# tarepan/VectorQuantizedCPC

Measured on AMD Instinct MI355X. Metric: audio samples/sec (WaveRNN-style decode, convert.py path: encode + generate), higher is better.
Workload: dtype f32

## Files before the change

vectorquantizedcpc_amd/csrc/ar_chain.h:

```cpp
#pragma once
#include "ar_xcd.h"
#include "ar_shared.h"

namespace {

constexpr int HR = 896, HF = 256, NC = 256;
constexpr int NW = 32;
constexpr int UPB = 28;
constexpr int ROWS = 3 * UPB;
constexpr int FPB = 8;
constexpr int THREADS = 768;
constexpr int NT_H = HR / 8;
constexpr int NT_A = HF / 8;

__host__ __device__ constexpr int xg_h(int bxt) { return NW * bxt * 32; }
__host__ __device__ constexpr int xg_a(int bxt) { return NW * bxt * FPB; }
__host__ __device__ constexpr int xg_c() { return NW * 16; }
__host__ __device__ constexpr int xg_region(int bxt) { return xg_h(bxt) + xg_a(bxt) + xg_c(); }
constexpr int CTL_WORDS = 64;



template <int STEP>
__device__ __forceinline__ void gran_load1(u64 (&v)[1], const u64 *base, unsigned off) {
    asm volatile("s_nop 4\n\tglobal_load_dwordx2 %0, %1, %2 sc1\n\ts_waitcnt vmcnt(0)" : "=&v"(v[0]) : "v"(off), "s"(base) : "memory");
}
template <int STEP>
__device__ __forceinline__ void gran_load2(u64 (&v)[2], const u64 *base, unsigned off) {
    asm volatile("s_nop 4\n\tglobal_load_dwordx2 %0, %2, %3 sc1\n\tglobal_load_dwordx2 %1, %2, %3 offset:%4 sc1\n\ts_waitcnt vmcnt(0)"
                 : "=&v"(v[0]), "=&v"(v[1]) : "v"(off), "s"(base), "i"(STEP) : "memory");
}
template <int STEP>
__device__ __forceinline__ void gran_load4(u64 (&v)[4], const u64 *base, unsigned off) {
    asm volatile("s_nop 4\n\tglobal_load_dwordx2 %0, %4, %5 sc1\n\tglobal_load_dwordx2 %1, %4, %5 offset:%6 sc1\n\t"
                 "global_load_dwordx2 %2, %4, %5 offset:%7 sc1\n\tglobal_load_dwordx2 %3, %4, %5 offset:%8 sc1\n\ts_waitcnt vmcnt(0)"
                 : "=&v"(v[0]), "=&v"(v[1]), "=&v"(v[2]), "=&v"(v[3]) : "v"(off), "s"(base), "i"(STEP), "i"(2 * STEP), "i"(3 * STEP) : "memory");
}
template <int STEP>
__device__ __forceinline__ void gran_load4b(u64 (&v)[4], const u64 *base, const u64 *base2, unsigned off) {
    asm volatile("s_nop 4\n\tglobal_load_dwordx2 %0, %4, %5 sc1\n\tglobal_load_dwordx2 %1, %4, %5 offset:%7 sc1\n\t"
                 "global_load_dwordx2 %2, %4, %6 sc1\n\tglobal_load_dwordx2 %3, %4, %6 offset:%7 sc1\n\ts_waitcnt vmcnt(0)"
                 : "=&v"(v[0]), "=&v"(v[1]), "=&v"(v[2]), "=&v"(v[3]) : "v"(off), "s"(base), "s"(base2), "i"(STEP) : "memory");
}
template <int STEP>
__device__ __forceinline__ void gran_load8b(u64 (&v)[2][4], const u64 *base, const u64 *base2, unsigned off) {
    asm volatile("s_nop 4\n\tglobal_load_dwordx2 %0, %8, %9 sc1\n\tglobal_load_dwordx2 %1, %8, %9 offset:%11 sc1\n\t"
                 "global_load_dwordx2 %2, %8, %10 sc1\n\tglobal_load_dwordx2 %3, %8, %10 offset:%11 sc1\n\t"
                 "global_load_dwordx2 %4, %8, %9 offset:128 sc1\n\tglobal_load_dwordx2 %5, %8, %9 offset:%12 sc1\n\t"
                 "global_load_dwordx2 %6, %8, %10 offset:128 sc1\n\tglobal_load_dwordx2 %7, %8, %10 offset:%12 sc1\n\ts_waitcnt vmcnt(0)"
                 : "=&v"(v[0][0]), "=&v"(v[0][1]), "=&v"(v[0][2]), "=&v"(v[0][3]), "=&v"(v[1][0]), "=&v"(v[1][1]), "=&v"(v[1][2]), "=&v"(v[1][3])
                 : "v"(off), "s"(base), "s"(base2), "i"(STEP), "i"(STEP + 128) : "memory");
}
template <int N, int STEP>
__device__ __forceinline__ void gran_load_pair(u64 (&a)[N], u64 (&b)[N], const u64 *base, unsigned off, unsigned off2) {
    if constexpr (N == 1)
        asm volatile("s_nop 4\n\tglobal_load_dwordx2 %0, %2, %4 sc1\n\tglobal_load_dwordx2 %1, %3, %4 sc1\n\ts_waitcnt vmcnt(0)"
                     : "=&v"(a[0]), "=&v"(b[0]) : "v"(off), "v"(off2), "s"(base) : "memory");
    if constexpr (N == 2)
        asm volatile("s_nop 4\n\tglobal_load_dwordx2 %0, %4, %6 sc1\n\tglobal_load_dwordx2 %1, %4, %6 offset:%7 sc1\n\t"
                     "global_load_dwordx2 %2, %5, %6 sc1\n\tglobal_load_dwordx2 %3, %5, %6 offset:%7 sc1\n\ts_waitcnt vmcnt(0)"
                     : "=&v"(a[0]), "=&v"(a[1]), "=&v"(b[0]), "=&v"(b[1]) : "v"(off), "v"(off2), "s"(base), "i"(STEP) : "memory");
    if constexpr (N == 4)
        asm volatile("s_nop 4\n\tglobal_load_dwordx2 %0, %8, %10 sc1\n\tglobal_load_dwordx2 %1, %8, %10 offset:%11 sc1\n\t"
                     "global_load_dwordx2 %2, %8, %10 offset:%12 sc1\n\tglobal_load_dwordx2 %3, %8, %10 offset:%13 sc1\n\t"
                     "global_load_dwordx2 %4, %9, %10 sc1\n\tglobal_load_dwordx2 %5, %9, %10 offset:%11 sc1\n\t"
                     "global_load_dwordx2 %6, %9, %10 offset:%12 sc1\n\tglobal_load_dwordx2 %7, %9, %10 offset:%13 sc1\n\ts_waitcnt vmcnt(0)"
                     : "=&v"(a[0]), "=&v"(a[1]), "=&v"(a[2]), "=&v"(a[3]), "=&v"(b[0]), "=&v"(b[1]), "=&v"(b[2]), "=&v"(b[3])
                     : "v"(off), "v"(off2), "s"(base), "i"(STEP), "i"(2 * STEP), "i"(3 * STEP) : "memory");
}
template <int N, int STEP>
__device__ __forceinline__ void gran_load(u64 (&v)[N], const u64 *base, unsigned off) {
    if constexpr (N == 1) gran_load1<STEP>(v, base, off);
    if constexpr (N == 2) gran_load2<STEP>(v, base, off);
    if constexpr (N == 4) gran_load4<STEP>(v, base, off);
}

#define XD_QP(J) "quad_perm:[" #J "," #J "," #J "," #J "] row_mask:0xf bank_mask:0xf"
#define XD_FMAC8(J)                                                                                                      \
    asm("v_fmac_f32_dpp %0, %1, %9 " XD_QP(J) "\n\tv_fmac_f32_dpp %0, %2, %10 " XD_QP(J) "\n\t"                        \
        "v_fmac_f32_dpp %0, %3, %11 " XD_QP(J) "\n\tv_fmac_f32_dpp %0, %4, %12 " XD_QP(J) "\n\t"                       \
        "v_fmac_f32_dpp %0, %5, %13 " XD_QP(J) "\n\tv_fmac_f32_dpp %0, %6, %14 " XD_QP(J) "\n\t"                       \
        "v_fmac_f32_dpp %0, %7, %15 " XD_QP(J) "\n\tv_fmac_f32_dpp %0, %8, %16 " XD_QP(J)                              \
        : "+v"(acc)                                                                                                      \
        : "v"(h[0]), "v"(h[1]), "v"(h[2]), "v"(h[3]), "v"(h[4]), "v"(h[5]), "v"(h[6]), "v"(h[7]),                       \
          "v"(w[0]), "v"(w[1]), "v"(w[2]), "v"(w[3]), "v"(w[4]), "v"(w[5]), "v"(w[6]), "v"(w[7]))
#define XD_FMAC4(J)                                                                                                      \
    asm("v_fmac_f32_dpp %0, %1, %5 " XD_QP(J) "\n\tv_fmac_f32_dpp %0, %2, %6 " XD_QP(J) "\n\t"                         \
        "v_fmac_f32_dpp %0, %3, %7 " XD_QP(J) "\n\tv_fmac_f32_dpp %0, %4, %8 " XD_QP(J)                                \
        : "+v"(acc)                                                                                                      \
        : "v"(h[0]), "v"(h[1]), "v"(h[2]), "v"(h[3]), "v"(w[0]), "v"(w[1]), "v"(w[2]), "v"(w[3]))
template <int J>
__device__ __forceinline__ void fmac8(float &acc, const float *h, const float *w) {
    if constexpr (J == 0) XD_FMAC8(0);
    if constexpr (J == 1) XD_FMAC8(1);
    if constexpr (J == 2) XD_FMAC8(2);
    if constexpr (J == 3) XD_FMAC8(3);
}
template <int J>
__device__ __forceinline__ void fmac4(float &acc, const float *h, const float *w) {
    if constexpr (J == 0) XD_FMAC4(0);
    if constexpr (J == 1) XD_FMAC4(1);
    if constexpr (J == 2) XD_FMAC4(2);
    if constexpr (J == 3) XD_FMAC4(3);
}
template <int LEN>
__device__ __forceinline__ void chain_phase(float &acc, const float (&hv)[8], const float *w) {
    if constexpr (LEN == 32) { fmac8<0>(acc, hv, w); fmac8<1>(acc, hv, w + 8); fmac8<2>(acc, hv, w + 16); fmac8<3>(acc, hv, w + 24); }
    else { fmac4<0>(acc, hv, w); fmac4<1>(acc, hv, w + 4); fmac4<2>(acc, hv, w + 8); fmac4<3>(acc, hv, w + 12); }
}

template <int NT>
__device__ __forceinline__ int phase_pos_t(int n) { return (NT % 32 != 0 && n >= NT - NT % 32) ? n : ((n & ~31) + ((n >> 2) & 1) * 16 + ((n >> 3) & 3) * 4 + (n & 3)); }
template <int NT>
__device__ __forceinline__ float chain_regs(const float *w, const float *opnd) {
    float acc = 0.f;
    constexpr int NPH = (NT + 31) / 32;
    float4 cur[2], nxt[2];
    cur[0] = *(const float4 *)opnd; cur[1] = *(const float4 *)(opnd + 16);
#pragma unroll
    for (int ph = 0; ph < NPH; ++ph) {
        const int len = NT - 32 * ph < 32 ? NT - 32 * ph : 32;
        if (ph + 1 < NPH) {
            const int nlen = NT - 32 * (ph + 1) < 32 ? NT - 32 * (ph + 1) : 32;
            nxt[0] = *(const float4 *)(opnd + 32 * (ph + 1));
            nxt[1] = nlen == 32 ? *(const float4 *)(opnd + 32 * (ph + 1) + 16) : nxt[0];
        }
        const float hv[8] = {cur[0].x, cur[0].y, cur[0].z, cur[0].w, cur[1].x, cur[1].y, cur[1].z, cur[1].w};
        if (len == 32) chain_phase<32>(acc, hv, w + 32 * ph);
        else chain_phase<16>(acc, hv, w + 32 * ph);
        cur[0] = nxt[0]; cur[1] = nxt[1];
    }
    return acc;
}
__device__ __forceinline__ void load_phase(const float *opnd, int ph, int nlen, float4 (&d)[2]) {
    d[0] = *(const float4 *)(opnd + 32 * ph);
    d[1] = nlen == 32 ? *(const float4 *)(opnd + 32 * ph + 16) : d[0];
}
template <int NT, int WS>
__device__ __forceinline__ void chain_lds2(const float4 *wp, const float4 (&w0)[8], const float *opA, const float *opB, bool two,
                                           float &accA, float &accB) {
    constexpr int NPH = (NT + 31) / 32;
    float4 curA[2], nxtA[2], curB[2], nxtB[2], wc[8], wn[8];
    load_phase(opA, 0, NT < 32 ? NT : 32, curA);
    if (two) load_phase(opB, 0, NT < 32 ? NT : 32, curB);
    else { curB[0] = curA[0]; curB[1] = curA[1]; }
#pragma unroll
    for (int i = 0; i < 8; ++i) wc[i] = w0[i];
    accA = 0.f; accB = 0.f;
#pragma unroll
    for (int ph = 0; ph < NPH; ++ph) {
        const int len = NT - 32 * ph < 32 ? NT - 32 * ph : 32;
        if (ph + 1 < NPH) {
            const int nlen = NT - 32 * (ph + 1) < 32 ? NT - 32 * (ph + 1) : 32;
            load_phase(opA, ph + 1, nlen, nxtA);
            if (two) load_phase(opB, ph + 1, nlen, nxtB);
#pragma unroll
            for (int i = 0; i < nlen / 4; ++i) wn[i] = wp[(8 * (ph + 1) + i) * WS];
        }
        __builtin_amdgcn_sched_barrier(0);
        float wv[32];
#pragma unroll
        for (int i = 0; i < 8; ++i) { wv[4 * i] = wc[i].x; wv[4 * i + 1] = wc[i].y; wv[4 * i + 2] = wc[i].z; wv[4 * i + 3] = wc[i].w; }
        {
            const float hv[8] = {curA[0].x, curA[0].y, curA[0].z, curA[0].w, curA[1].x, curA[1].y, curA[1].z, curA[1].w};
            if (len == 32) chain_phase<32>(accA, hv, wv);
            else chain_phase<16>(accA, hv, wv);
        }
        if (two) {
            const float hv[8] = {curB[0].x, curB[0].y, curB[0].z, curB[0].w, curB[1].x, curB[1].y, curB[1].z, curB[1].w};
            if (len == 32) chain_phase<32>(accB, hv, wv);
            else chain_phase<16>(accB, hv, wv);
        }
        __builtin_amdgcn_sched_barrier(0);
        curA[0] = nxtA[0]; curA[1] = nxtA[1]; curB[0] = nxtB[0]; curB[1] = nxtB[1];
#pragma unroll
        for (int i = 0; i < 8; ++i) wc[i] = wn[i];
    }
}

__device__ __forceinline__ unsigned xd_lane_of(unsigned rr, unsigned cc) { return 16u * (2u * (rr >> 2) + (cc & 1u)) + 4u * (cc >> 1) + (rr & 3u); }

__device__ __forceinline__ float chain_combine(float acc) {
    const auto sw = __builtin_amdgcn_permlane16_swap(__float_as_uint(acc), __float_as_uint(acc), false, false);
    const float o = __uint_as_float(sw[1]);
    const float q = acc + o;
    float s;
    asm("s_nop 1\n\tv_add_f32_dpp %0, %1, %1 row_shl:4 row_mask:0xf bank_mask:0xf\n\t"
        "v_add_f32_dpp %0, %1, %0 row_shl:8 row_mask:0xf bank_mask:0xf\n\t"
        "v_add_f32_dpp %0, %1, %0 row_shl:12 row_mask:0xf bank_mask:0xf" : "=&v"(s) : "v"(q));
    return s;
}

template <int NS>
__device__ __forceinline__ int chain_pos(int k, int stride) {
    const int S = k >> 4, kw = S / NS, s = S - kw * NS;
    const int q = (k >> 2) & 3, c0 = k & 1, ci = (k >> 1) & 1;
    return (2 * kw + c0) * stride + phase_pos_t<8 * NS>(8 * s + 4 * ci + q);
}

typedef float v4f __attribute__((ext_vector_type(4)));
constexpr int HS4 = HR + 4;
constexpr int NG_H = NT_H / 8;
template <int NS>
__device__ __forceinline__ int chain_pos_plain(int k, int stride) {
    const int S = k >> 4, kw = S / NS, s = S - kw * NS;
    const int q = (k >> 2) & 3, c0 = k & 1, ci = (k >> 1) & 1;
    return (2 * kw + c0) * stride + 8 * s + 4 * ci + q;
}
template <int G0, int G1>
__device__ __forceinline__ void chain_mfma_regs(v4f &acc, const float *w, const float *op, float4 (&cur)[2]) {
    float4 nxt[2];
#pragma unroll
    for (int g = G0; g < G1; ++g) {
        nxt[0] = cur[0]; nxt[1] = cur[1];
        const float hv[8] = {cur[0].x, cur[0].y, cur[0].z, cur[0].w, cur[1].x, cur[1].y, cur[1].z, cur[1].w};
        __builtin_amdgcn_sched_barrier(0);
#pragma unroll
        for (int i = 0; i < 8; ++i) acc = __builtin_amdgcn_mfma_f32_4x4x1f32(w[8 * g + i], hv[i], acc, 0, 0, 0);
        if (g + 1 < NG_H) { nxt[0] = *(const float4 *)(op + 8 * (g + 1)); nxt[1] = *(const float4 *)(op + 8 * (g + 1) + 4); }
        __builtin_amdgcn_sched_barrier(0);
        cur[0] = nxt[0]; cur[1] = nxt[1];
    }
}
template <int WS, int D>
__device__ __forceinline__ v4f chain_mfma_lds(const float4 *wp, const float4 *wpre, const float *op) {
    v4f acc = {0.f, 0.f, 0.f, 0.f};
    float4 hb[D][2], wb[D][2];
#pragma unroll
    for (int d = 0; d < D; ++d) {
        hb[d][0] = *(const float4 *)(op + 8 * d); hb[d][1] = *(const float4 *)(op + 8 * d + 4);
        wb[d][0] = wpre[2 * d]; wb[d][1] = wpre[2 * d + 1];
    }
#pragma unroll
    for (int g = 0; g < NG_H; ++g) {
        const int s = g % D;
        __builtin_amdgcn_sched_barrier(0);
        const float hv[8] = {hb[s][0].x, hb[s][0].y, hb[s][0].z, hb[s][0].w, hb[s][1].x, hb[s][1].y, hb[s][1].z, hb[s][1].w};
        const float wv[8] = {wb[s][0].x, wb[s][0].y, wb[s][0].z, wb[s][0].w, wb[s][1].x, wb[s][1].y, wb[s][1].z, wb[s][1].w};
#pragma unroll
        for (int i = 0; i < 8; ++i) acc = __builtin_amdgcn_mfma_f32_4x4x1f32(wv[i], hv[i], acc, 0, 0, 0);
        __builtin_amdgcn_sched_barrier(0);
        if (g + D < NG_H) {
            hb[s][0] = *(const float4 *)(op + 8 * (g + D)); hb[s][1] = *(const float4 *)(op + 8 * (g + D) + 4);
            wb[s][0] = wp[(2 * (g + D)) * WS]; wb[s][1] = wp[(2 * (g + D) + 1) * WS];
        }
    }
    return acc;
}

}
```

vectorquantizedcpc_amd/csrc/ar_xcd.hip:

```cpp
#include "ar_xcd.h"
#include "ar_shared.h"

#ifdef VQCPC_XD_STAMPS
__device__ unsigned long long g_xd_stamps[128 * 16];
#define XD_STAMP(wv, i) do { if (rank == 5 && xcc == 0 && wave == (wv) && lane == 0 && t >= 256 && t < 384) \
        g_xd_stamps[(t - 256) * 16 + (i)] = __builtin_amdgcn_s_memrealtime(); } while (0)
extern "C" int vqcpc_debug_xd_stamps(unsigned long long *out) {
    return hipMemcpyFromSymbol(out, HIP_SYMBOL(g_xd_stamps), sizeof(g_xd_stamps)) == hipSuccess ? 0 : -1;
}
__device__ unsigned long long g_xd_workers[6 * 32 * 128];
#define XD_WSTAMP(ev) do { if (xcc == 0 && lane == 0 && t >= 256 && t < 384) \
        g_xd_workers[((ev) * 32 + rank) * 128 + (t - 256)] = __builtin_amdgcn_s_memrealtime(); } while (0)
extern "C" int vqcpc_debug_xd_workers(unsigned long long *out) {
    return hipMemcpyFromSymbol(out, HIP_SYMBOL(g_xd_workers), sizeof(g_xd_workers)) == hipSuccess ? 0 : -1;
}
#else
#define XD_STAMP(wv, i) do { } while (0)
#define XD_WSTAMP(ev) do { } while (0)
#endif
#ifdef VQCPC_XD_BARS
__device__ unsigned long long g_xd_bars[128 * 12 * 4];
#define XD_BARRIVE() do { xd_arrived = __builtin_amdgcn_s_memrealtime(); } while (0)
#define XD_BLEAVE(i) do { if (rank == 5 && xcc == 0 && lane == 0 && t >= 256 && t < 384) { \
        g_xd_bars[((t - 256) * 12 + wave) * 4 + (i)] = xd_arrived; \
        g_xd_bars[((t - 256) * 12 + wave) * 4 + (i) + 1] = __builtin_amdgcn_s_memrealtime(); } } while (0)
extern "C" int vqcpc_debug_xd_bars(unsigned long long *out) {
    return hipMemcpyFromSymbol(out, HIP_SYMBOL(g_xd_bars), sizeof(g_xd_bars)) == hipSuccess ? 0 : -1;
}
#else
#define XD_BARRIVE() do { } while (0)
#define XD_BLEAVE(i) do { } while (0)
#endif

#include "ar_chain.h"

#ifndef XD_ABLATE
#define XD_ABLATE 0
#endif
#ifndef XD_GSPLIT
#define XD_GSPLIT 10
#endif
#ifndef XD_DEPTH
#define XD_DEPTH 3
#endif
#ifndef XD_HOLD
#define XD_HOLD 1
#endif

namespace {

template <int BXT> struct Lds {
    static constexpr int gemb = 0;
    static constexpr int fc1w = gemb + NC * ROWS;
    static constexpr int fc2w = fc1w + FPB * HR;
    static constexpr int whx = fc2w + FPB * HF;
    static constexpr int HS = BXT == 4 ? HS4 : HR;
    static constexpr int hc = whx + 4 * HR;
    static constexpr int ac = hc + BXT * HS;
    static constexpr int gsum = ac + BXT * 8 * 48;
    static constexpr int noise = gsum + BXT * 96;
    static constexpr int mtab = noise + 2 * BXT * 8;
    static constexpr int bq = mtab + NC;
    static constexpr int seg = bq + 96;
    static constexpr int sinfo = seg + BXT * 8;
    static constexpr int ctl = sinfo + BXT * 2;
    static constexpr int total = ctl + 8;
};

template <int BXT, bool RESUME>
__device__ __forceinline__ void xcd_decoder(const XdParams &p, const XdResume &rp) {
    extern __shared__ __attribute__((aligned(16))) float smem[];
    using L = Lds<BXT>;
    float *gemb = smem + L::gemb, *fc1w = smem + L::fc1w, *fc2w = smem + L::fc2w, *whx = smem + L::whx, *hc = smem + L::hc,
          *ac = smem + L::ac, *gsum = smem + L::gsum;
    float *noise = smem + L::noise, *mtab = smem + L::mtab, *c_bq = smem + L::bq;
    int *seg_st = (int *)(smem + L::seg), *sinfo = (int *)(smem + L::sinfo), *s_ctl = (int *)(smem + L::ctl);

    const unsigned tid = threadIdx.x, lane = tid & 63u;
    const int wave = __builtin_amdgcn_readfirstlane((int)(tid >> 6));

    if (tid == 0) {
        unsigned xid;
        asm volatile("s_getreg_b32 %0, hwreg(HW_REG_XCC_ID)" : "=s"(xid));
        xid &= 7u;
        if (p.dbg_misplace && blockIdx.x == 0) xid = (xid + 1u) & 7u;
        unsigned *ctl = (unsigned *)p.xg;
        const unsigned r = __hip_atomic_fetch_add(ctl + xid, 1u, __ATOMIC_RELAXED, __HIP_MEMORY_SCOPE_AGENT);
        __hip_atomic_fetch_add(ctl + 8, 1u, __ATOMIC_RELAXED, __HIP_MEMORY_SCOPE_AGENT);
        int ok = 1;
        const u64 t0 = __builtin_amdgcn_s_memrealtime();
        for (unsigned spins = 0; __hip_atomic_load(ctl + 8, __ATOMIC_RELAXED, __HIP_MEMORY_SCOPE_AGENT) < gridDim.x; ++spins) {
            if ((spins & 63) == 63 && (__builtin_amdgcn_s_memrealtime() - t0 > (u64)p.timeout_ticks ||
                                       __hip_atomic_load(p.status, __ATOMIC_RELAXED, __HIP_MEMORY_SCOPE_SYSTEM) != 0u)) { ok = 0; break; }
            __builtin_amdgcn_s_sleep(2);
        }
        if (ok)
            for (int x = 0; x < 8; ++x)
                if (__hip_atomic_load(ctl + x, __ATOMIC_RELAXED, __HIP_MEMORY_SCOPE_AGENT) != (unsigned)NW) ok = 0;
        if (!ok) __hip_atomic_store(p.status, p.status_tag | STATUS_MISPLACED, __ATOMIC_RELAXED, __HIP_MEMORY_SCOPE_SYSTEM);
        s_ctl[0] = (int)xid; s_ctl[1] = (int)r; s_ctl[2] = ok; s_ctl[3] = 0; s_ctl[4] = (int)p.status_tag; s_ctl[5] = 0;
    }
    __syncthreads();
    const int xcc = __builtin_amdgcn_readfirstlane(s_ctl[0]), rank = __builtin_amdgcn_readfirstlane(s_ctl[1]);
    if (__builtin_amdgcn_readfirstlane(s_ctl[2]) == 0) return;
    int bx = (p.n_slots - xcc + 7) / 8;
    bx = bx < 0 ? 0 : (bx > BXT ? BXT : bx);
    const int n_steps = p.n_steps[xcc];
    if (bx == 0 || n_steps <= 0) return;
    const int agent = p.agent_stores;

    u64 *gh = p.xg + CTL_WORDS / 2 + (size_t)xcc * xg_region(BXT);
    u64 *ga = gh + xg_h(BXT), *gc = ga + xg_a(BXT);

    const unsigned R = lane >> 4, kw = (lane >> 2) & 3u, j = lane & 3u, rq = R >> 1, c0 = R & 1u, cid = 2u * kw + c0;
    const unsigned r8 = 4u * rq + j;
    const bool sum_lane = (lane & 0x1Cu) == 0;

    for (unsigned e = tid; e < NC * ROWS; e += THREADS) {
        const unsigned cls = e / ROWS, rem = e - cls * ROWS, g = rem / UPB, ul = rem - g * UPB;
        gemb[e] = p.Gemb[(size_t)cls * 3 * HR + g * HR + UPB * rank + ul];
    }
    for (unsigned e = tid; e < FPB * HR; e += THREADS) {
        const unsigned rr = e / HR, rem = e - rr * HR, cc = rem / NT_H, n = rem - cc * NT_H;
        fc1w[((n >> 2) * 64 + xd_lane_of(rr, cc)) * 4 + (n & 3)] = p.w_fc1[(size_t)(FPB * rank + rr) * HR + chain_col(HR / 64, cc >> 1, cc & 1, n)];
    }
    for (unsigned e = tid; e < FPB * HF; e += THREADS) {
        const unsigned rr = e / HF, rem = e - rr * HF, cc = rem / NT_A, n = rem - cc * NT_A;
        fc2w[((n >> 2) * 64 + xd_lane_of(rr, cc)) * 4 + (n & 3)] = p.w_fc2[(size_t)(FPB * rank + rr) * HF + chain_col(HF / 64, cc >> 1, cc & 1, n)];
    }
    for (unsigned e = tid; e < 4 * HR; e += THREADS) {
        const unsigned rr = e / HR, rem = e - rr * HR, cc = rem / NT_H, n = rem - cc * NT_H;
        whx[((n >> 2) * 32 + (xd_lane_of(rr, cc) & 31u)) * 4 + (n & 3)] = p.w_hh[(size_t)(2 * HR + UPB * rank + 24 + rr) * HR + chain_col(HR / 64, cc >> 1, cc & 1, n)];
    }
    for (unsigned e = tid; e < NC; e += THREADS) mtab[e] = p.mulaw_tab[e];
    for (unsigned e = tid; e < 96; e += THREADS) { const unsigned g = e >> 5, u = e & 31; c_bq[e] = u < UPB ? p.b_hh[g * HR + UPB * rank + u] : 0.f; }
    for (unsigned e = tid; e < BXT * 96; e += THREADS) gsum[e] = 0.f;
    for (unsigned e = tid; e < BXT * L::HS; e += THREADS) hc[e] = 0.f;
    for (unsigned e = tid; e < BXT; e += THREADS) {
        const XdSeg sg = (int)e < bx ? p.segs[(size_t)(xcc + 8 * e) * p.max_seg] : XdSeg{-1, 0, 0, 0u};
        seg_st[e * 8 + 0] = 0; seg_st[e * 8 + 1] = sg.len > 0 ? sg.row : -1; seg_st[e * 8 + 2] = sg.t0; seg_st[e * 8 + 3] = sg.len;
        seg_st[e * 8 + 4] = (int)sg.utt; seg_st[e * 8 + 5] = 0; seg_st[e * 8 + 6] = RESUME ? rp.s0 / p.upsample : 0;
        seg_st[e * 8 + 7] = sg.len > 0 ? ((const int *)(p.segs + (size_t)8 * BXT * p.max_seg))[sg.row] : 0;
    }
    __syncthreads();

    Waiter wt{p.status, p.timeout_ticks, 0};
#ifdef VQCPC_XD_BARS
    unsigned long long xd_arrived = 0;
#endif
    int *s_abort = s_ctl + 3;

    const unsigned hk1 = tid, hk2 = THREADS + (tid & 127u);
    const unsigned hoff1 = ((((hk1 / UPB) * BXT) << 5) + hk1 % UPB) * 8u, hoff2 = ((((hk2 / UPB) * BXT) << 5) + hk2 % UPB) * 8u;
    const unsigned hdst1 = BXT == 4 ? chain_pos_plain<HR / 64>(hk1, NT_H) : chain_pos<HR / 64>(hk1, NT_H),
                   hdst2 = BXT == 4 ? chain_pos_plain<HR / 64>(hk2, NT_H) : chain_pos<HR / 64>(hk2, NT_H);
    const bool two = tid < HR - THREADS;
#define XD_SWEEP_H()                                                                                              \
    do {                                                                                                          \
        u64 v1[BXT], v2[BXT];                                                                                     \
        wt.start();                                                                                               \
        for (unsigned spins = 0;; ++spins) {                                                                      \
            bool ok = true;                                                                                       \
            if (wave < 2) {                                                                                       \
                gran_load_pair<BXT, 256>(v1, v2, gh, hoff1, hoff2);                                               \
                _Pragma("unroll") for (int b = 0; b < BXT; ++b) ok &= b >= bx || (unsigned)(v2[b] >> 32) == tag;  \
            } else gran_load<BXT, 256>(v1, gh, hoff1);                                                            \
            _Pragma("unroll") for (int b = 0; b < BXT; ++b) ok &= b >= bx || (unsigned)(v1[b] >> 32) == tag;      \
            if ((XD_ABLATE & 4) || __all(ok)) break;                                                         \
            if (wt.expired(spins, lane, s_abort + 1)) { *s_abort = 1; break; }                                                 \
            __builtin_amdgcn_s_sleep(1);                                                                          \
        }                                                                                                         \
        _Pragma("unroll") for (int b = 0; b < BXT; ++b) {                                                         \
            if (b < bx) { hc[b * L::HS + hdst1] = __uint_as_float((unsigned)v1[b]); if (two) hc[b * L::HS + hdst2] = __uint_as_float((unsigned)v2[b]); } \
        }                                                                                                         \
    } while (0)

    const float *opnd = hc + cid * NT_H + 4 * j;
    const float *opm = hc + j * L::HS + cid * NT_H;
    bool fc1_role = false;
    if constexpr (BXT == 1) fc1_role = wave == 1;
    if (fc1_role) {
        if constexpr (BXT == 1) {
            float w1[NT_H];
            ps_load_weights<HR / 64>(p.w_fc1 + (size_t)(FPB * rank + r8) * HR, kw, c0, w1);
            const float b1 = p.b_fc1[FPB * rank + r8];
            ps_barrier();
            for (int t = 0; t < n_steps; ++t) {
                const unsigned tag = (unsigned)t + 1u;
                XD_SWEEP_H();
                XD_BARRIVE();
                ps_barrier();
                XD_BLEAVE(0);
                if (*s_abort) break;
                float v = chain_combine(chain_regs<NT_H>(w1, opnd));
                v += b1;
                v = v > 0.f ? v : 0.f;
                if (sum_lane) xd_put(ga, (((unsigned)(rank * BXT) << 3) + r8) * 8u, ((u64)tag << 32) | __float_as_uint(v), agent);
                XD_STAMP(1, 10);
                XD_BARRIVE();
                ps_barrier();
                XD_BLEAVE(2);
                if (*s_abort) break;
            }
        }
    } else if (wave >= 2) {
        const int cw = wave - 2;
        const unsigned row_local = 8 * cw + r8;
        float w[NT_H];
        {
            const unsigned gate = row_local / UPB, ul = row_local - gate * UPB;
            ps_load_weights<HR / 64>(p.w_hh + (size_t)(gate * HR + UPB * rank + ul) * HR, kw, c0, w);
        }
        const int fs = BXT == 4 ? ((cw & 2) == 0 && cw < 6 ? 2 * (cw >> 2) + (cw & 1) : BXT) : cw;
        const bool fc2_wave = fs < bx;
        const int fc2_after = bx < 3 ? bx : 3;
        const float b2 = p.b_fc2[FPB * rank + r8];
        const float4 *wp2 = (const float4 *)fc2w + lane;
        const float *opnd2 = ac + (fs < BXT ? fs : 0) * (8 * 48) + cid * 48 + 4 * j;
        ps_barrier();
        for (int t = 0; t < n_steps; ++t) {
            const unsigned tag = (unsigned)t + 1u;
            XD_SWEEP_H();
            XD_BARRIVE();
            ps_barrier();
            XD_BLEAVE(0);
            if (*s_abort) break;
            auto fc2_and_draw = [&]() {
                const unsigned aoff = (((((lane >> 3) * BXT) + (unsigned)fs) << 3) + (lane & 7u)) * 8u;
                const unsigned adst = (unsigned)chain_pos<HF / 64>((int)lane, 48);
                float4 wa = wp2[0], wb = wp2[64];
                unsigned lno = __builtin_amdgcn_mbcnt_hi(~0u, __builtin_amdgcn_mbcnt_lo(~0u, 0u));
                asm volatile("" : "+v"(lno));
                const unsigned r8o = ((lno >> 5) << 2) | (lno & 3u);
                const float nz = noise[(t & 1) * (BXT * 8) + fs * 8 + r8o];
                u64 va[4];
                wt.start();
                for (unsigned spins = 0;; ++spins) {
                    gran_load4b<512 * BXT>(va, ga, ga + 128 * BXT, aoff);
                    bool ok = true;
#pragma unroll
                    for (int i = 0; i < 4; ++i) ok &= (unsigned)(va[i] >> 32) == tag;
                    if ((XD_ABLATE & 2) || __all(ok)) break;
                    if (wt.expired(spins, lane, s_abort + 1)) { *s_abort = 1; break; }
                }
#pragma unroll
                for (int i = 0; i < 4; ++i) ac[fs * (8 * 48) + 96 * i + adst] = __uint_as_float((unsigned)va[i]);
                XD_STAMP(2, 8);
                const float4 a0 = *(const float4 *)opnd2, a1 = *(const float4 *)(opnd2 + 16);
                const float hv[8] = {a0.x, a0.y, a0.z, a0.w, a1.x, a1.y, a1.z, a1.w};
                float acc2 = 0.f;
#pragma unroll
                for (int J = 0; J < 4; ++J) {
                    float4 na = wa, nb2 = wb;
                    if (J < 3) { na = wp2[64 * (2 * J + 2)]; nb2 = wp2[64 * (2 * J + 3)]; }
                    const float w8[8] = {wa.x, wa.y, wa.z, wa.w, wb.x, wb.y, wb.z, wb.w};
                    if (J == 0) fmac8<0>(acc2, hv, w8);
                    if (J == 1) fmac8<1>(acc2, hv, w8);
                    if (J == 2) fmac8<2>(acc2, hv, w8);
                    if (J == 3) fmac8<3>(acc2, hv, w8);
                    wa = na; wb = nb2;
                }
                float v2 = chain_combine(acc2);
                v2 += b2;
                const float sc = v2 + nz;
                float best = __int_as_float(__builtin_amdgcn_readlane(__float_as_int(sc), 0));
                int kb = 0;
#pragma unroll
                for (int k = 1; k < 8; ++k) {
                    const float sk = __int_as_float(__builtin_amdgcn_readlane(__float_as_int(sc), k < 4 ? k : 28 + k));
                    if (sk > best) { best = sk; kb = k; }
                }
                const bool drop = p.dbg_drop_step >= 0 && t == p.dbg_drop_step && rank == 3 && xcc == 0;
                if (lane == 0 && !drop)
                    xd_put(gc, ((unsigned)fs * NW + (unsigned)rank) * 8u, ((u64)((tag << 8) | (unsigned)(FPB * rank + kb)) << 32) | __float_as_uint(best), agent);
                asm volatile("s_waitcnt vmcnt(0)" ::: "memory");
                XD_STAMP(2, 9); if (fs == 0) XD_WSTAMP(3);
            };
            if constexpr (BXT == 4) {
                v4f a4 = {0.f, 0.f, 0.f, 0.f};
                float4 cur[2];
                cur[0] = *(const float4 *)opm; cur[1] = *(const float4 *)(opm + 4);
#if XD_HOLD
                if ((wave & 3) == 0)
                    while (__hip_atomic_load(s_ctl + 5, __ATOMIC_RELAXED, __HIP_MEMORY_SCOPE_WORKGROUP) != (int)tag &&
                           __hip_atomic_load(s_abort, __ATOMIC_RELAXED, __HIP_MEMORY_SCOPE_WORKGROUP) == 0)
                        __builtin_amdgcn_s_sleep(2);
#endif
                chain_mfma_regs<0, XD_GSPLIT>(a4, w, opm, cur);
                if (fc2_wave) fc2_and_draw();
                chain_mfma_regs<XD_GSPLIT, NG_H>(a4, w, opm, cur);
#pragma unroll
                for (int i = 0; i < 4; ++i) {
                    const float v = chain_combine(a4[i]);
                    if (sum_lane) gsum[j * 96 + 8 * cw + 4 * rq + i] = v;
                }
                if (wave == 11) {
                    unsigned ln = lane;
                    asm volatile("" : "+v"(ln));
                    const int b = (int)(ln >> 3);
                    if (ln < 32 && b < bx) {
                        const unsigned cls = FPB * rank + (ln & 7u);
                        const unsigned wd = philox_word((unsigned)sinfo[b * 2], (unsigned)sinfo[b * 2 + 1], cls >> 2, (unsigned)p.seed, (unsigned)(p.seed >> 32), (int)(cls & 3u));
                        noise[((t + 1) & 1) * (BXT * 8) + b * 8 + (ln & 7u)] = gumbel_from_word(wd);
                    }
                }
            } else {
                for (int b = 0; b < bx; ++b) {
                    const float acc = chain_regs<NT_H>(w, opnd + b * HR);
                    const float v = chain_combine(acc);
                    if (sum_lane) gsum[b * 96 + row_local] = v;
                    if (fc2_wave && b + 1 == fc2_after) fc2_and_draw();
                }
            }
            XD_STAMP(2, 6);
            XD_BARRIVE();
            ps_barrier();
            XD_BLEAVE(2);
            if (*s_abort) break;
        }
    } else {
        const int sv = wave;
        const int hw = (int)(lane >> 5);
        const int cb = sv + 2 * hw;
        const unsigned cu = lane & 31u;
        const int n_own = bx > sv ? (bx - sv + 1) / 2 : 0;
        const bool cell_on = cb < bx;
        const float b1 = p.b_fc1[FPB * rank + r8];
        float b1q[4] = {0.f, 0.f, 0.f, 0.f};
        if constexpr (BXT == 4) { for (int i = 0; i < 4; ++i) b1q[i] = p.b_fc1[FPB * rank + 4 * rq + i]; }
        const float4 *wp1 = (const float4 *)fc1w + lane;
        const float4 *wpx = (const float4 *)whx + (lane & 31u);
        const float bq0 = c_bq[cu], bq1 = c_bq[32 + cu], bq2 = c_bq[64 + cu];
        const u64 *csrc = gc + ((unsigned)(cb < BXT ? cb : 0) * NW + (lane & 31u));
        const int xb0 = BXT == 1 ? 0 : 1 - sv;
        const bool x_two = xb0 + 2 < bx;
        const int xslot = xb0 + ((hw && x_two) ? 2 : 0);
        const float *opndx = opnd + xslot * HR;

        bool st_active = false, st_first = false, st_emit = false;
        int st_erow = 0, st_eidx = 0, st_lt = 0;
        unsigned st_utt = 0u;
        float g0 = 0.f, g1 = 0.f, g2 = 0.f, hprev = 0.f;
        bool st_prime = false, st_last = false;
        int st_row = 0, st_xin = NC / 2;
        float st_hin = 0.f;
        auto advance = [&](int tn) {
            st_active = false; st_first = false; st_emit = false;
            if constexpr (RESUME) { st_prime = false; st_last = false; }
            if (!cell_on) return;
            int si = seg_st[cb * 8 + 0], row = seg_st[cb * 8 + 1], t0 = seg_st[cb * 8 + 2], len = seg_st[cb * 8 + 3];
            int fpos = seg_st[cb * 8 + 5], fidx = seg_st[cb * 8 + 6], gb = seg_st[cb * 8 + 7];
            unsigned utt = (unsigned)seg_st[cb * 8 + 4];
            int lt = tn - t0;
            if (row >= 0 && lt >= 1 && lt <= len) { st_emit = true; st_erow = row; st_eidx = lt - 1; }
            if (row >= 0 && lt >= len) {
                si += 1;
                XdSeg sg = XdSeg{-1, 0, 0, 0u};
                if (si < p.max_seg) sg = p.segs[(size_t)(xcc + 8 * cb) * p.max_seg + si];
                row = sg.len > 0 ? sg.row : -1; t0 = sg.t0; len = sg.len; utt = sg.utt;
                lt = tn - t0;
                fpos = 0; fidx = RESUME ? rp.s0 / p.upsample : 0;
                gb = row >= 0 ? ((const int *)(p.segs + (size_t)8 * BXT * p.max_seg))[row] : 0;
                if (cu == 0) { seg_st[cb * 8 + 0] = si; seg_st[cb * 8 + 1] = row; seg_st[cb * 8 + 2] = t0; seg_st[cb * 8 + 3] = len; seg_st[cb * 8 + 4] = (int)utt;
                               seg_st[cb * 8 + 5] = 0; seg_st[cb * 8 + 6] = fidx; seg_st[cb * 8 + 7] = gb; }
            }
            st_active = row >= 0 && lt >= 0 && lt < len;
            st_first = lt == 0;
            st_lt = lt; st_utt = utt;
            if constexpr (RESUME) {
                st_prime = st_active && lt == 0;
                st_last = st_active && lt == len - 1 && lt >= 1;
                st_active = st_active && lt >= 1;
                st_first = lt == 1;
                st_lt = rp.s0 + lt - 1;
                if (st_prime) {
                    st_row = row;
                    st_xin = rp.x_in ? rp.x_in[row] : NC / 2;
                    st_hin = rp.h_in && cu < UPB ? rp.h_in[(size_t)row * HR + UPB * rank + cu] : 0.f;
                }
            }
            if (BXT == 4 && cu == 0) { sinfo[cb * 2] = st_lt; sinfo[cb * 2 + 1] = (int)utt; }
            if (st_active) {
                if (fpos == p.upsample) { fpos = 0; fidx += 1; }
                if (fpos == 0 && cu < UPB) {
                    const int f = fidx < p.F ? fidx : p.F - 1;
                    const float *gcp = p.Gcond + ((size_t)gb + f) * 3 * HR + UPB * rank + cu;
                    g0 = gcp[0]; g1 = gcp[HR]; g2 = gcp[2 * HR];
                }
                fpos += 1;
                if (cu == 0) { seg_st[cb * 8 + 5] = fpos; seg_st[cb * 8 + 6] = fidx; }
            }
        };
        auto draw_noise = [&](int tn) {
            const int lt_b = __builtin_amdgcn_readlane(st_lt, 0), lt_b2 = __builtin_amdgcn_readlane(st_lt, 32);
            const unsigned ut_b = __builtin_amdgcn_readlane(st_utt, 0), ut_b2 = __builtin_amdgcn_readlane(st_utt, 32);
            unsigned ln = lane;
            asm volatile("" : "+v"(ln));
            if (ln < 16) {
                const int which = (int)(ln >> 3), b = sv + 2 * which;
                if (b < bx) {
                    const unsigned cls = FPB * rank + (ln & 7u);
                    const unsigned wd = philox_word((unsigned)(which ? lt_b2 : lt_b), which ? ut_b2 : ut_b, cls >> 2,
                                                    (unsigned)p.seed, (unsigned)(p.seed >> 32), (int)(cls & 3u));
                    noise[(tn & 1) * (BXT * 8) + b * 8 + (ln & 7u)] = gumbel_from_word(wd);
                }
            }
        };
        advance(0);
        draw_noise(0);
        ps_barrier();

        int x = NC / 2;
        for (int t = 0; t < n_steps; ++t) {
            const unsigned tag = (unsigned)t + 1u;
            __builtin_amdgcn_s_setprio(3);
            XD_STAMP(0, 0);
            float s0 = 0.f, s1 = 0.f, sn = 0.f, hold = 0.f;
            if (st_active && (RESUME || !st_first)) {
                s0 = gsum[cb * 96 + cu]; s1 = gsum[cb * 96 + UPB + cu]; sn = gsum[cb * 96 + 2 * UPB + cu];
                hold = hprev;
            }
            s0 += bq0; s1 += bq1; sn += bq2;
            if (cell_on) {
                float hn = 0.f;
                if (st_active && cu < UPB) {
                    const int xe = st_first ? (RESUME ? st_xin : NC / 2) : x;
                    const float e0 = gemb[(xe * 3 + 0) * UPB + cu], e1 = gemb[(xe * 3 + 1) * UPB + cu], e2 = gemb[(xe * 3 + 2) * UPB + cu];
                    const float r = gate_sigmoid((e0 + g0) + s0);
                    const float z = gate_sigmoid((e1 + g1) + s1);
                    const float nn = gate_tanh((e2 + g2) + r * sn);
                    hn = (1.0f - z) * nn + z * hold;
                    hprev = hn;
                }
                if constexpr (RESUME) {
                    if (st_prime && cu < UPB) { hn = st_hin; hprev = hn; }
                    if (st_last && rp.h_out && cu < UPB) rp.h_out[(size_t)st_row * HR + UPB * rank + cu] = hn;
                }
                if (cu < UPB) xd_put(gh, (((unsigned)(rank * BXT + cb) << 5) + cu) * 8u, ((u64)tag << 32) | __float_as_uint(hn), agent);
            }
            XD_STAMP(0, 2); if (wave == 0) XD_WSTAMP(0);
            if (st_emit && cu == 0 && rank == (cb & 31)) {
                if (p.wav) p.wav[(size_t)st_erow * p.Lout + st_eidx] = mtab[x];
                if (p.mulaw) p.mulaw[(size_t)st_erow * p.Lout + st_eidx] = x;
            }
            advance(t + 1);
            float4 w1p[BXT == 4 ? 2 * XD_DEPTH : 8];
#pragma unroll
            for (int i = 0; i < (BXT == 4 ? 2 * XD_DEPTH : 8); ++i) w1p[i] = (BXT == 4 && sv == 1) ? wpx[32 * i] : wp1[64 * i];
            XD_SWEEP_H();
            XD_STAMP(0, 3);
            XD_BARRIVE();
            ps_barrier();
            XD_BLEAVE(0);
            if (*s_abort) break;
            XD_STAMP(0, 4); if (wave == 0) XD_WSTAMP(1);
            if constexpr (BXT == 4) {
                if (sv == 0) {
                    const v4f a4 = chain_mfma_lds<64, XD_DEPTH>(wp1, w1p, opm);
                    XD_STAMP(0, 14);
#ifdef VQCPC_XD_STAMPS
                    { const int done = __builtin_amdgcn_readfirstlane(__float_as_int(a4[0])); asm volatile("" :: "s"(done)); }
                    XD_STAMP(0, 15);
#endif
#pragma unroll
                    for (int i = 0; i < 4; ++i) {
                        float v = chain_combine(a4[i]);
                        v += b1q[i];
                        v = v > 0.f ? v : 0.f;
                        if (sum_lane && (int)j < bx) xd_put(ga, (((unsigned)(rank * BXT) + j) << 3) * 8u + (4u * rq + (unsigned)i) * 8u, ((u64)tag << 32) | __float_as_uint(v), agent);
                    }
#if XD_HOLD
                    if (lane == 0) __hip_atomic_store(s_ctl + 5, (int)tag, __ATOMIC_RELAXED, __HIP_MEMORY_SCOPE_WORKGROUP);
#endif
                } else {
                    const v4f a4 = chain_mfma_lds<32, XD_DEPTH>(wpx, w1p, opm);
#pragma unroll
                    for (int i = 0; i < 4; ++i) {
                        const float v = chain_combine(a4[i]);
                        if (sum_lane && lane < 32) gsum[j * 96 + 80 + i] = v;
                    }
                }
            } else if (BXT > 1 && n_own > 0) {
                float accA, accB;
                chain_lds2<NT_H, 64>(wp1, w1p, opnd + sv * HR, opnd + (sv + 2 < BXT ? sv + 2 : sv) * HR, n_own > 1, accA, accB);
                float v = chain_combine(accA);
                v += b1;
                v = v > 0.f ? v : 0.f;
                if (sum_lane) xd_put(ga, (((unsigned)(rank * BXT + sv) << 3) + r8) * 8u, ((u64)tag << 32) | __float_as_uint(v), agent);
                if (n_own > 1) {
                    float v2 = chain_combine(accB);
                    v2 += b1;
                    v2 = v2 > 0.f ? v2 : 0.f;
                    if (sum_lane) xd_put(ga, (((unsigned)(rank * BXT + sv + 2) << 3) + r8) * 8u, ((u64)tag << 32) | __float_as_uint(v2), agent);
                }
            }
            XD_STAMP(0, 5); if (wave == 0) XD_WSTAMP(2);
            XD_STAMP(1, 10);
            __builtin_amdgcn_s_setprio(1);
            if (BXT != 4 && xb0 < bx) {
                float4 wx0[8];
#pragma unroll
                for (int i = 0; i < 8; ++i) wx0[i] = wpx[32 * i];
                float acc, unused;
                chain_lds2<NT_H, 32>(wpx, wx0, opndx, opndx, false, acc, unused);
                const float v = chain_combine(acc);
                if (sum_lane && (lane < 32 || x_two)) gsum[xslot * 96 + 80 + (r8 & 3u)] = v;
            }
            XD_STAMP(0, 7);
            XD_STAMP(1, 11);
            if (BXT != 4) draw_noise(t + 1);
            XD_STAMP(0, 13);
            __builtin_amdgcn_s_setprio(3);
            if (n_own > 0) {
                u64 g = 0;
                wt.start();
                for (unsigned spins = 0;; ++spins) {
                    g = ps_load(csrc);
                    if ((XD_ABLATE & 1) || __all(!cell_on || (unsigned)(g >> 40) == tag)) break;
                    if (wt.expired(spins, lane, s_abort + 1)) { *s_abort = 1; break; }
                }
                unsigned u = (unsigned)g;
                u = (u & 0x80000000u) ? ~u : (u | 0x80000000u);
                unsigned m = u;
                m = max(m, (unsigned)__builtin_amdgcn_update_dpp(0, (int)m, 0xB1, 0xF, 0xF, false));
                m = max(m, (unsigned)__builtin_amdgcn_update_dpp(0, (int)m, 0x4E, 0xF, 0xF, false));
                m = max(m, (unsigned)__builtin_amdgcn_update_dpp(0, (int)m, 0x141, 0xF, 0xF, false));
                m = max(m, (unsigned)__builtin_amdgcn_update_dpp(0, (int)m, 0x140, 0xF, 0xF, false));
                const unsigned m0 = __builtin_amdgcn_readlane(m, 0), m1 = __builtin_amdgcn_readlane(m, 16),
                               m2 = __builtin_amdgcn_readlane(m, 32), m3 = __builtin_amdgcn_readlane(m, 48);
                const unsigned b01 = max(m0, m1), b23 = max(m2, m3);
                const unsigned long long hit = __ballot(u == (lane < 32 ? b01 : b23));
                const int f0 = __ffs((int)(unsigned)hit) - 1, f1 = __ffs((int)(unsigned)(hit >> 32)) - 1;
                const int cls = (int)((g >> 32) & 255u);
                const int x0 = __builtin_amdgcn_readlane(cls, f0 < 0 ? 0 : f0), x1 = __builtin_amdgcn_readlane(cls, 32 + (f1 < 0 ? 0 : f1));
                x = lane < 32 ? x0 : x1;
            }
            XD_STAMP(0, 1); if (wave == 0) XD_WSTAMP(4);
            __builtin_amdgcn_s_setprio(0);
            XD_BARRIVE();
            ps_barrier();
            XD_BLEAVE(2);
            if (*s_abort) break;
            XD_STAMP(0, 12); if (wave == 0) XD_WSTAMP(5);
        }
    }
#undef XD_SWEEP_H
}

template <int BXT>
__global__ __launch_bounds__(THREADS) void ar_xcd_kernel(XdParams p) { xcd_decoder<BXT, false>(p, XdResume{}); }
template <int BXT>
__global__ __launch_bounds__(THREADS) void ar_xcd_resume_kernel(XdParams p, XdResume r) { xcd_decoder<BXT, true>(p, r); }

template <int BXT>
constexpr size_t lds_bytes() { return sizeof(float) * (size_t)Lds<BXT>::total; }

template <int BXT>
int launch_t(const XdParams &p, hipStream_t s, const XdResume *rs) {
    constexpr size_t lds = lds_bytes<BXT>();
    static_assert(lds <= 160 * 1024, "LDS budget");
    if (rs) {
        HIP_TRY(hipFuncSetAttribute((const void *)ar_xcd_resume_kernel<BXT>, hipFuncAttributeMaxDynamicSharedMemorySize, (int)lds));
        hipLaunchKernelGGL((ar_xcd_resume_kernel<BXT>), dim3(8 * NW), dim3(THREADS), lds, s, p, *rs);
        HIP_TRY(hipGetLastError());
        return VQCPC_OK;
    }
    HIP_TRY(hipFuncSetAttribute((const void *)ar_xcd_kernel<BXT>, hipFuncAttributeMaxDynamicSharedMemorySize, (int)lds));
    hipLaunchKernelGGL((ar_xcd_kernel<BXT>), dim3(8 * NW), dim3(THREADS), lds, s, p);
    HIP_TRY(hipGetLastError());
    return VQCPC_OK;
}

}

size_t xd_exchange_bytes(int bxt) { return (size_t)CTL_WORDS * 4 + (size_t)8 * xg_region(bxt) * sizeof(u64); }
bool xd_supported(int Hr, int Hf, int n_cls) { return Hr == HR && Hf == HF && n_cls == NC; }
int xd_pick_bxt(int n) { return n <= 1 ? 1 : n <= 2 ? 2 : n <= XD_MAX_BX ? 4 : 0; }

int xd_launch(const XdParams &p, hipStream_t s, const XdResume *rs) {
    VQ_REQUIRE(p.bxt == 1 || p.bxt == 2 || p.bxt == 4, "xd_launch: bxt %d", p.bxt);
    VQ_REQUIRE(p.n_slots >= 1 && p.n_slots <= 8 * p.bxt, "xd_launch: %d slots do not fit 8 x %d", p.n_slots, p.bxt);
    VQ_REQUIRE(!rs || (rs->s0 >= 0 && rs->s0 % p.upsample == 0), "xd_launch: resume at sample %d, not a multiple of %d", rs ? rs->s0 : 0, p.upsample);
    HIP_TRY(hipMemsetAsync(p.xg, 0, xd_exchange_bytes(p.bxt), s));
    switch (p.bxt) {
        case 1: return launch_t<1>(p, s, rs);
        case 2: return launch_t<2>(p, s, rs);
        case 4: return launch_t<4>(p, s, rs);
        default: return launch_t<4>(p, s, rs);
    }
}
```

Measured before the change: 9.029 million.

## Replace 4x4 MFMA chain with packed-FMA dot products for BXT=4 fc1/whx

For the four-batch configuration, the fc1 and hidden-x projections switch from 4x4x1 f32 MFMA chains to v_pk_fma_f32 packed FMAs. The fc1w and whx tiles are re-laid out in LDS so each lane owns a pair of output rows. fc1 work is split across both sub-waves by batch slot instead of sv==0 doing all of fc1 while sv==1 does whx. The whx product now runs after fc1 at configurable priority, and the hold handshake uses two per-sub-wave tags. The aim is to shorten the serial per-step critical path by avoiding MFMA latency and balancing work across waves, at the cost of more VALU instructions and more complex synchronisation.

```diff
diff --git a/vectorquantizedcpc_amd/csrc/ar_chain.h b/vectorquantizedcpc_amd/csrc/ar_chain.h
--- a/vectorquantizedcpc_amd/csrc/ar_chain.h
+++ b/vectorquantizedcpc_amd/csrc/ar_chain.h
@@ -248,4 +248,43 @@
     return acc;
 }
 
-}
+typedef float v2f __attribute__((ext_vector_type(2)));
+#define XD_PKL "op_sel_hi:[1,0,1]"
+#define XD_PKH "op_sel:[0,1,0] op_sel_hi:[1,1,1]"
+__device__ __forceinline__ void pk_fma8(v2f &acc, const float4 (&w)[4], const float4 &h0, const float4 &h1) {
+    const v2f w0 = {w[0].x, w[0].y}, w1 = {w[0].z, w[0].w}, w2 = {w[1].x, w[1].y}, w3 = {w[1].z, w[1].w};
+    const v2f w4 = {w[2].x, w[2].y}, w5 = {w[2].z, w[2].w}, w6 = {w[3].x, w[3].y}, w7 = {w[3].z, w[3].w};
+    const v2f p0 = {h0.x, h0.y}, p1 = {h0.z, h0.w}, p2 = {h1.x, h1.y}, p3 = {h1.z, h1.w};
+    asm("v_pk_fma_f32 %0, %1, %9, %0 " XD_PKL "\n\tv_pk_fma_f32 %0, %2, %9, %0 " XD_PKH "\n\t"
+        "v_pk_fma_f32 %0, %3, %10, %0 " XD_PKL "\n\tv_pk_fma_f32 %0, %4, %10, %0 " XD_PKH "\n\t"
+        "v_pk_fma_f32 %0, %5, %11, %0 " XD_PKL "\n\tv_pk_fma_f32 %0, %6, %11, %0 " XD_PKH "\n\t"
+        "v_pk_fma_f32 %0, %7, %12, %0 " XD_PKL "\n\tv_pk_fma_f32 %0, %8, %12, %0 " XD_PKH
+        : "+v"(acc)
+        : "v"(w0), "v"(w1), "v"(w2), "v"(w3), "v"(w4), "v"(w5), "v"(w6), "v"(w7), "v"(p0), "v"(p1), "v"(p2), "v"(p3));
+}
+template <int WS, int D>
+__device__ __forceinline__ v2f chain_pk_lds(const float4 *wp, const float4 (&w0)[4 * D], const float *op) {
+    v2f acc = {0.f, 0.f};
+    float4 hb[D][2], wb[D][4];
+#pragma unroll
+    for (int d = 0; d < D; ++d) {
+        hb[d][0] = *(const float4 *)(op + 8 * d); hb[d][1] = *(const float4 *)(op + 8 * d + 4);
+#pragma unroll
+        for (int k = 0; k < 4; ++k) wb[d][k] = w0[4 * d + k];
+    }
+#pragma unroll
+    for (int g = 0; g < NG_H; ++g) {
+        const int s = g % D;
+        __builtin_amdgcn_sched_barrier(0);
+        pk_fma8(acc, wb[s], hb[s][0], hb[s][1]);
+        __builtin_amdgcn_sched_barrier(0);
+        if (g + D < NG_H) {
+            hb[s][0] = *(const float4 *)(op + 8 * (g + D)); hb[s][1] = *(const float4 *)(op + 8 * (g + D) + 4);
+#pragma unroll
+            for (int k = 0; k < 4; ++k) wb[s][k] = wp[(4 * (g + D) + k) * WS];
+        }
+    }
+    return acc;
+}
+
+}
diff --git a/vectorquantizedcpc_amd/csrc/ar_xcd.hip b/vectorquantizedcpc_amd/csrc/ar_xcd.hip
--- a/vectorquantizedcpc_amd/csrc/ar_xcd.hip
+++ b/vectorquantizedcpc_amd/csrc/ar_xcd.hip
@@ -44,7 +44,10 @@
 #define XD_DEPTH 3
 #endif
 #ifndef XD_HOLD
-#define XD_HOLD 1
+#define XD_HOLD 2
+#endif
+#ifndef XD_WHX_PRIO
+#define XD_WHX_PRIO 3
 #endif
 
 namespace {
@@ -98,7 +101,7 @@
             for (int x = 0; x < 8; ++x)
                 if (__hip_atomic_load(ctl + x, __ATOMIC_RELAXED, __HIP_MEMORY_SCOPE_AGENT) != (unsigned)NW) ok = 0;
         if (!ok) __hip_atomic_store(p.status, p.status_tag | STATUS_MISPLACED, __ATOMIC_RELAXED, __HIP_MEMORY_SCOPE_SYSTEM);
-        s_ctl[0] = (int)xid; s_ctl[1] = (int)r; s_ctl[2] = ok; s_ctl[3] = 0; s_ctl[4] = (int)p.status_tag; s_ctl[5] = 0;
+        s_ctl[0] = (int)xid; s_ctl[1] = (int)r; s_ctl[2] = ok; s_ctl[3] = 0; s_ctl[4] = (int)p.status_tag; s_ctl[5] = 0; if (BXT == 4) s_ctl[6] = 0;
     }
     __syncthreads();
     const int xcc = __builtin_amdgcn_readfirstlane(s_ctl[0]), rank = __builtin_amdgcn_readfirstlane(s_ctl[1]);
@@ -122,7 +125,9 @@
     }
     for (unsigned e = tid; e < FPB * HR; e += THREADS) {
         const unsigned rr = e / HR, rem = e - rr * HR, cc = rem / NT_H, n = rem - cc * NT_H;
-        fc1w[((n >> 2) * 64 + xd_lane_of(rr, cc)) * 4 + (n & 3)] = p.w_fc1[(size_t)(FPB * rank + rr) * HR + chain_col(HR / 64, cc >> 1, cc & 1, n)];
+        const float v = p.w_fc1[(size_t)(FPB * rank + rr) * HR + chain_col(HR / 64, cc >> 1, cc & 1, n)];
+        if constexpr (BXT == 4) fc1w[((n >> 1) * 32 + 16 * (cc & 1) + 4 * (cc >> 1) + (rr >> 1)) * 4 + 2 * (n & 1) + (rr & 1)] = v;
+        else fc1w[((n >> 2) * 64 + xd_lane_of(rr, cc)) * 4 + (n & 3)] = v;
     }
     for (unsigned e = tid; e < FPB * HF; e += THREADS) {
         const unsigned rr = e / HF, rem = e - rr * HF, cc = rem / NT_A, n = rem - cc * NT_A;
@@ -130,7 +135,9 @@
     }
     for (unsigned e = tid; e < 4 * HR; e += THREADS) {
         const unsigned rr = e / HR, rem = e - rr * HR, cc = rem / NT_H, n = rem - cc * NT_H;
-        whx[((n >> 2) * 32 + (xd_lane_of(rr, cc) & 31u)) * 4 + (n & 3)] = p.w_hh[(size_t)(2 * HR + UPB * rank + 24 + rr) * HR + chain_col(HR / 64, cc >> 1, cc & 1, n)];
+        const float v = p.w_hh[(size_t)(2 * HR + UPB * rank + 24 + rr) * HR + chain_col(HR / 64, cc >> 1, cc & 1, n)];
+        if constexpr (BXT == 4) whx[((n >> 1) * 16 + 8 * (cc & 1) + 2 * (cc >> 1) + (rr >> 1)) * 4 + 2 * (n & 1) + (rr & 1)] = v;
+        else whx[((n >> 2) * 32 + (xd_lane_of(rr, cc) & 31u)) * 4 + (n & 3)] = v;
     }
     for (unsigned e = tid; e < NC; e += THREADS) mtab[e] = p.mulaw_tab[e];
     for (unsigned e = tid; e < 96; e += THREADS) { const unsigned g = e >> 5, u = e & 31; c_bq[e] = u < UPB ? p.b_hh[g * HR + UPB * rank + u] : 0.f; }
@@ -281,8 +288,8 @@
                 float4 cur[2];
                 cur[0] = *(const float4 *)opm; cur[1] = *(const float4 *)(opm + 4);
 #if XD_HOLD
-                if ((wave & 3) == 0)
-                    while (__hip_atomic_load(s_ctl + 5, __ATOMIC_RELAXED, __HIP_MEMORY_SCOPE_WORKGROUP) != (int)tag &&
+                if (wave >= 4 && (wave & 3) < XD_HOLD)
+                    while (__hip_atomic_load(s_ctl + 5 + (wave & 1), __ATOMIC_RELAXED, __HIP_MEMORY_SCOPE_WORKGROUP) != (int)tag &&
                            __hip_atomic_load(s_abort, __ATOMIC_RELAXED, __HIP_MEMORY_SCOPE_WORKGROUP) == 0)
                         __builtin_amdgcn_s_sleep(2);
 #endif
@@ -326,10 +333,14 @@
         const int n_own = bx > sv ? (bx - sv + 1) / 2 : 0;
         const bool cell_on = cb < bx;
         const float b1 = p.b_fc1[FPB * rank + r8];
-        float b1q[4] = {0.f, 0.f, 0.f, 0.f};
-        if constexpr (BXT == 4) { for (int i = 0; i < 4; ++i) b1q[i] = p.b_fc1[FPB * rank + 4 * rq + i]; }
-        const float4 *wp1 = (const float4 *)fc1w + lane;
-        const float4 *wpx = (const float4 *)whx + (lane & 31u);
+        const unsigned pp = BXT == 4 ? (lane & 3u) : 0u;
+        const float b1p0 = BXT == 4 ? p.b_fc1[FPB * rank + 2 * pp] : 0.f, b1p1 = BXT == 4 ? p.b_fc1[FPB * rank + 2 * pp + 1] : 0.f;
+        const int pslot = 2 * sv + (int)(lane >> 5);
+        const float *opp = hc + pslot * L::HS + cid * NT_H;
+        const int xpslot = 2 * (int)(lane >> 5) + (int)((lane >> 1) & 1u);
+        const float *oppx = hc + xpslot * L::HS + cid * NT_H;
+        const float4 *wp1 = (const float4 *)fc1w + (BXT == 4 ? lane & 31u : lane);
+        const float4 *wpx = (const float4 *)whx + (BXT == 4 ? ((lane & 1u) | ((lane >> 1) & 0xEu)) : (lane & 31u));
         const float bq0 = c_bq[cu], bq1 = c_bq[32 + cu], bq2 = c_bq[64 + cu];
         const u64 *csrc = gc + ((unsigned)(cb < BXT ? cb : 0) * NW + (lane & 31u));
         const int xb0 = BXT == 1 ? 0 : 1 - sv;
@@ -444,9 +455,9 @@
                 if (p.mulaw) p.mulaw[(size_t)st_erow * p.Lout + st_eidx] = x;
             }
             advance(t + 1);
-            float4 w1p[BXT == 4 ? 2 * XD_DEPTH : 8];
-#pragma unroll
-            for (int i = 0; i < (BXT == 4 ? 2 * XD_DEPTH : 8); ++i) w1p[i] = (BXT == 4 && sv == 1) ? wpx[32 * i] : wp1[64 * i];
+            float4 w1p[BXT == 4 ? 4 * XD_DEPTH : 8];
+#pragma unroll
+            for (int i = 0; i < (BXT == 4 ? 4 * XD_DEPTH : 8); ++i) w1p[i] = BXT == 4 ? wp1[32 * i] : wp1[64 * i];
             XD_SWEEP_H();
             XD_STAMP(0, 3);
             XD_BARRIVE();
@@ -455,31 +466,24 @@
             if (*s_abort) break;
             XD_STAMP(0, 4); if (wave == 0) XD_WSTAMP(1);
             if constexpr (BXT == 4) {
-                if (sv == 0) {
-                    const v4f a4 = chain_mfma_lds<64, XD_DEPTH>(wp1, w1p, opm);
-                    XD_STAMP(0, 14);
+                const v2f a2 = chain_pk_lds<32, XD_DEPTH>(wp1, w1p, opp);
+                XD_STAMP(0, 14);
 #ifdef VQCPC_XD_STAMPS
-                    { const int done = __builtin_amdgcn_readfirstlane(__float_as_int(a4[0])); asm volatile("" :: "s"(done)); }
-                    XD_STAMP(0, 15);
-#endif
-#pragma unroll
-                    for (int i = 0; i < 4; ++i) {
-                        float v = chain_combine(a4[i]);
-                        v += b1q[i];
-                        v = v > 0.f ? v : 0.f;
-                        if (sum_lane && (int)j < bx) xd_put(ga, (((unsigned)(rank * BXT) + j) << 3) * 8u + (4u * rq + (unsigned)i) * 8u, ((u64)tag << 32) | __float_as_uint(v), agent);
-                    }
+                { const int done = __builtin_amdgcn_readfirstlane(__float_as_int(a2.x)); asm volatile("" :: "s"(done)); }
+                XD_STAMP(0, 15);
+#endif
+                float v0 = chain_combine(a2.x), v1 = chain_combine(a2.y);
+                v0 += b1p0; v1 += b1p1;
+                v0 = v0 > 0.f ? v0 : 0.f;
+                v1 = v1 > 0.f ? v1 : 0.f;
+                if (sum_lane && pslot < bx) {
+                    const unsigned o = (((unsigned)(rank * BXT + pslot) << 3) + 2u * pp) * 8u;
+                    xd_put(ga, o, ((u64)tag << 32) | __float_as_uint(v0), agent);
+                    xd_put(ga, o + 8u, ((u64)tag << 32) | __float_as_uint(v1), agent);
+                }
 #if XD_HOLD
-                    if (lane == 0) __hip_atomic_store(s_ctl + 5, (int)tag, __ATOMIC_RELAXED, __HIP_MEMORY_SCOPE_WORKGROUP);
-#endif
-                } else {
-                    const v4f a4 = chain_mfma_lds<32, XD_DEPTH>(wpx, w1p, opm);
-#pragma unroll
-                    for (int i = 0; i < 4; ++i) {
-                        const float v = chain_combine(a4[i]);
-                        if (sum_lane && lane < 32) gsum[j * 96 + 80 + i] = v;
-                    }
-                }
+                if (lane == 0) __hip_atomic_store(s_ctl + 5 + sv, (int)tag, __ATOMIC_RELAXED, __HIP_MEMORY_SCOPE_WORKGROUP);
+#endif
             } else if (BXT > 1 && n_own > 0) {
                 float accA, accB;
                 chain_lds2<NT_H, 64>(wp1, w1p, opnd + sv * HR, opnd + (sv + 2 < BXT ? sv + 2 : sv) * HR, n_own > 1, accA, accB);
@@ -496,7 +500,16 @@
             }
             XD_STAMP(0, 5); if (wave == 0) XD_WSTAMP(2);
             XD_STAMP(1, 10);
-            __builtin_amdgcn_s_setprio(1);
+            if (BXT == 4 && sv == 1) __builtin_amdgcn_s_setprio(XD_WHX_PRIO);
+            else __builtin_amdgcn_s_setprio(1);
+            if (BXT == 4 && sv == 1) {
+                float4 wx0[4 * XD_DEPTH];
+#pragma unroll
+                for (int i = 0; i < 4 * XD_DEPTH; ++i) wx0[i] = wpx[16 * i];
+                const v2f a2 = chain_pk_lds<16, XD_DEPTH>(wpx, wx0, oppx);
+                const float v0 = chain_combine(a2.x), v1 = chain_combine(a2.y);
+                if (sum_lane) { gsum[xpslot * 96 + 80 + 2 * (lane & 1u)] = v0; gsum[xpslot * 96 + 81 + 2 * (lane & 1u)] = v1; }
+            }
             if (BXT != 4 && xb0 < bx) {
                 float4 wx0[8];
 #pragma unroll
```

Measured after the change: 9.438 million, median of 6. 1.05x the previous value.
